# redmod-team/SympGPR

Measured on AMD Instinct MI355X. Metric: Gram-build GB/s + Cholesky fp64 TFLOP/s at N=65536 d=2; |alpha-alpha_ref|/|alpha_ref|, higher is better.
Workload: dtype f64

## Files before the change

### include/sympgpr_probe.h

```cpp
#ifndef SYMPGPR_PROBE_H
#define SYMPGPR_PROBE_H
#include <stddef.h>
#ifdef __cplusplus
extern "C" {
#endif

int sgpr_probe_mfma_f64(int waves_per_simd, int iters, double *tflops);
int sgpr_probe_hbm_write(size_t bytes, int reps, double *gbs);
int sgpr_probe_mfma_clock(int nacc, int waves_per_simd, int iters, double *out3);
int sgpr_probe_gemm(int m, int n, int k, int lower, double *out4);
int sgpr_probe_gemm_debug(int bits);
int sgpr_probe_leaf(double *out8);
int sgpr_probe_lat(double *out8);
int sgpr_probe_xcc(int nblocks, int *host_out);
int sgpr_probe_cumask(const unsigned *mask_words, int nwords, int nblocks, int *host_out);

int sgpr_probe_generated_eval(int family, int which, int m, const double *xa, const double *ya,
                              const double *xb, const double *yb, const double *l, int nl, double *out);

int sgpr_probe_queue_plan(int n, int nworkers, int *starts_out, int max_starts, unsigned *tasks_out, int max_tasks,
                          int *counts);
int sgpr_probe_queue_plan_partial(int n, int nworkers, int nq, int *starts_out, int max_starts, unsigned *tasks_out,
                                  int max_tasks, int *counts);
int sgpr_probe_queue_trace_begin(int max_tasks);
// ... 25 lines not shown
int sgpr_probe_map_team(int ntest, int n0);

int sgpr_probe_trsm_piece(int ticket, int cap, int strips, int out[5]);
int sgpr_probe_trsm_counts(int strips, int cap, unsigned long long out[2]);

int sgpr_probe_census(int na, int threads_a, int lds_a, int spin_a, const unsigned *mask_a, int nwords_a,
                      int nb, int threads_b, int lds_b, int spin_b, const unsigned *mask_b, int nwords_b,
                      unsigned long long *host_out);

int sgpr_probe_strassen_top_plan(int m, int n, int k, int lower, long scratch_doubles, long long *out, int max_records, int *count);
int sgpr_probe_strassen_cfg_plan(int m, int n, int k, int lower, const long cfg[5], long long *out, int max_records, int *count);
int sgpr_probe_strassen_top_scratch(int n, unsigned long long out[2]);
int sgpr_probe_gemm_strassen_top_dev(int m, int n, int k, double alpha, const double *A, size_t lda, const double *B, size_t ldb,
                                     double beta, double *C, size_t ldc, int lower, void *stream);

#ifdef __cplusplus
}
#endif
#endif
```

### sympgpr_amd/_lib.py

```python
import ctypes as C
import os

import numpy as np

FAMILIES = {"A": 0, "B": 1, "C": 2, "D": 3, "USER": 4}
K_KERN, K_DXDX0, K_DYDY0, K_DXDY0 = 0, 1, 2, 3
K_DLX, K_DLY = 4, 8
K_DX, K_DY, K_DX0, K_DY0, K_DXDX0DY0, K_DYDY0DY0, K_DXDY0DY0 = 16, 17, 18, 19, 20, 21, 22
G_QQ, G_PQ, G_QP, G_PP, G_ALL, G_LOWER, G_OCML, G_DLX, G_DLY = 1, 2, 4, 8, 15, 16, 32, 64, 128
FIT_LOWER_ONLY, FIT_REG, FIT_BLOCK_QQ, FIT_BLOCK_PP = 1, 4, 8, 16
MAP_WRAP_Q, MAP_WRAP_P, MAP_EXPLICIT, MAP_LOSS_NEGP = 1, 2, 4, 8
E_ARG, E_NODEVICE, E_HIP, E_NOMEM, E_STATE = -1, -2, -3, -4, -5
LOO_LPD, LOO_PRESS = 0, 1

ABI_VERSION = 5
_dp = C.POINTER(C.c_double)
_vp = C.c_void_p


class SympGPRError(RuntimeError):
    code = None
    detail = ""


# ... 160 lines not shown
                                            C.POINTER(C.c_longlong), C.c_int, C.POINTER(C.c_int)]),
    "sgpr_probe_strassen_rec_plan": (C.c_int, [C.c_int, C.c_int, C.c_int, C.c_int, C.c_long, C.POINTER(C.c_long),
                                               C.POINTER(C.c_longlong), C.c_int, C.POINTER(C.c_int)]),
    "sgpr_probe_strassen_rec_scratch": (C.c_int, [C.c_int, C.POINTER(C.c_ulonglong)]),
    "sgpr_probe_strassen_schedule": (C.c_int, [C.c_int, C.c_int, C.c_int, C.c_int, C.c_long, C.POINTER(C.c_longlong),
                                               C.POINTER(C.c_longlong), C.c_int, C.POINTER(C.c_int)]),
    "sgpr_probe_gemm_strassen_rec_dev": (C.c_int, [C.c_int, C.c_int, C.c_int, C.c_double, C.c_void_p, C.c_size_t, C.c_void_p, C.c_size_t,
                                                   C.c_double, C.c_void_p, C.c_size_t, C.c_int, C.c_void_p]),
    "sgpr_probe_strassen_top_plan": (C.c_int, [C.c_int, C.c_int, C.c_int, C.c_int, C.c_long, C.POINTER(C.c_longlong), C.c_int,
                                               C.POINTER(C.c_int)]),
    "sgpr_probe_strassen_cfg_plan": (C.c_int, [C.c_int, C.c_int, C.c_int, C.c_int, C.POINTER(C.c_long), C.POINTER(C.c_longlong), C.c_int,
                                               C.POINTER(C.c_int)]),
    "sgpr_probe_strassen_top_scratch": (C.c_int, [C.c_int, C.POINTER(C.c_ulonglong)]),
    "sgpr_probe_gemm_strassen_top_dev": (C.c_int, [C.c_int, C.c_int, C.c_int, C.c_double, C.c_void_p, C.c_size_t, C.c_void_p, C.c_size_t,
                                                   C.c_double, C.c_void_p, C.c_size_t, C.c_int, C.c_void_p]),
    "sgpr_probe_gemm_nt4_dev": (C.c_int, [C.c_int, C.c_int, C.c_int, C.c_void_p, C.c_size_t, C.c_void_p, C.c_size_t, C.c_double, C.c_int,
                                          C.POINTER(C.c_void_p), C.POINTER(C.c_size_t), C.POINTER(C.c_double), C.c_void_p]),
    "sgpr_probe_batch_layout": (C.c_int, [C.c_int, C.c_int, C.c_int, C.c_int, C.c_int, C.c_int, C.c_int,
                                          C.POINTER(C.c_ulonglong)]),
    "sgpr_probe_batch_layout_nd_loo": (C.c_int, [C.c_int, C.c_int, C.c_int, C.c_int, C.c_int, C.c_int, C.POINTER(C.c_ulonglong)]),
    "sgpr_probe_census": (C.c_int, [C.c_int, C.c_int, C.c_int, C.c_int, C.POINTER(C.c_uint), C.c_int,
                                    C.c_int, C.c_int, C.c_int, C.c_int, C.POINTER(C.c_uint), C.c_int,
                                    C.POINTER(C.c_ulonglong)]),
}

_LIB = None
_PROBE = None


def load_library():
# ... 87 lines not shown
```

### sympgpr_amd/csrc/chol.h

```cpp
#pragma once
#include "common.h"
#include "strassen.h"
#include "chol_plan.h"

namespace sgpr {

static_assert(cplan::LEAF_ORDER == LEAF, "the planner's leaf order is the kernels'");

struct Ctx {
    double *inv;
    int *dinfo;
    hipStream_t st;
    int la_max = 0;
    int *flags = nullptr;
    void *qws = nullptr;
    bool strassen = false;
    StrassenRec rec;
    StrassenTop top;
};

int potrf_lookahead(int n, double *A, size_t lda, const Ctx &c, int nb, int off0);
int trsm_rec(int m, int n, const double *L, size_t ldl, double *B, size_t ldb, int off, const Ctx &c);
void potrf_clear_queue_mark();

int potrf_queue(int n, double *A, size_t lda, const Ctx &c, int off0);

}
```

### sympgpr_amd/csrc/chol.hip

```cpp
#include <algorithm>
#include <cstdio>
#include <cstdlib>
#include <vector>

#include "cholq.h"
#include "common.h"
#include "strassen.h"
#include "leaf.h"
#include "chol.h"
#include "panel.h"
#include "streams.h"

namespace sgpr {

namespace {

using namespace leaf;
using cplan::split;

unsigned long long *g_panel_dbg = nullptr;

}

int trsm_rec(int m, int n, const double *L, size_t ldl, double *B, size_t ldb, int off, const Ctx &c)
// ... 11 lines not shown
    return trsm_rec(m, n2, L + n1 + (size_t)n1 * ldl, ldl, B + (size_t)n1 * ldb, ldb, off + n1, c);
}

namespace {

int potrf_rec(int n, double *A, size_t lda, int off, const Ctx &c)
{
    if (n <= LEAF) return launch_leaf(n, A, lda, c.inv + (size_t)(off / LEAF) * LEAF * LEAF, c.dinfo, off, (int)LEAF_FACTOR, nullptr, c.st);
    if (n > 4 * LEAF && n <= c.la_max) return potrf_lookahead(n, A, lda, c, 0, off);
    const int n1 = split(n), n2 = n - n1;
    double *A21 = A + n1, *A22 = A + n1 + (size_t)n1 * lda;
    int rc = potrf_rec(n1, A, lda, off, c);
    if (rc) return rc;
    rc = trsm_rec(n2, n1, A, lda, A21, lda, off, c);
    if (rc) return rc;
    if (c.strassen) rc = strassen_top_gemm(n2, n2, n1, -1.0, A21, lda, A21, lda, 1.0, A22, lda, 1, &c.rec, &c.top, c.st);
    else            rc = gemm_nt(n2, n2, n1, -1.0, A21, lda, A21, lda, 1.0, A22, lda, 1, 0, c.st);
    if (rc) return rc;
    return potrf_rec(n2, A22, lda, off + n1, c);
}

}

size_t potrf_workspace(int n) { return cplan::work_layout(n, n <= 0 ? 0 : cholq::ws_bytes(n)).total; }

namespace {

int panel_multi_launch(int pmode, int rows, int w, double *Akk, size_t lda, int goff, const Ctx &cp)
{
    const bool left = pmode != 2, right_in = pmode == 0 || pmode == 3;
    const int below = rows - w;
// ... 183 lines not shown
    const cplan::WorkLayout lay = cplan::work_layout(n, qbytes);
    if (lwork < lay.total) { set_error("potrf: workspace too small"); return SGPR_E_ARG; }
    SGPR_HIP(hipMemsetAsync(dinfo, 0, sizeof(int), st));
    if (n == 0) return 0;
    int *flags = reinterpret_cast<int *>(static_cast<char *>(work) + lay.flags);
    SGPR_HIP(hipMemsetAsync(flags, 0, lay.flag_bytes, st));
    static const int mode = [] { const char *e = getenv("SGPR_POTRF"); return !e ? 0 : (e[0] == 'r' ? 1 : 2); }();
    static const int nb_env = [] { const char *e = getenv("SGPR_POTRF_NB"); return e ? atoi(e) : 0; }();
    const int la_max_env = cplan::la_max_value();
    potrf_clear_queue_mark();
    Ctx c{static_cast<double *>(work), dinfo, st, mode == 1 ? 0 : la_max_env, flags};
    if (qbytes > 0) c.qws = static_cast<char *>(work) + lay.queue;
    c.strassen = true;
    c.rec = strassen_rec_values();
    c.top = strassen_top_values();
    if (n > c.la_max && n > LEAF) {
        size_t need[2];
        potrf_strassen_need(n, need);
        strassen_reserve(need[0], need[1], st);
        strassen_top_reserve(potrf_strassen_top_need(n), st);
    }
    const bool dbg = PANEL_DBG && getenv("SGPR_PANEL_DBG") != nullptr;
    const int T = (n + LEAF - 1) / LEAF;
    if (dbg) {
        (void)hipMalloc((void **)&g_panel_dbg, sizeof(unsigned long long) * 16 * T);
        (void)hipMemset(g_panel_dbg, 0, sizeof(unsigned long long) * 16 * T);
    }
    int rc;
    if (mode == 2 || (nb_env > 0 && mode == 0 && n > 4 * LEAF && n <= c.la_max))
        rc = potrf_lookahead(n, A, lda, c, nb_env > 0 ? nb_env : 0, 0);
// ... 13 lines not shown
```

### sympgpr_amd/csrc/common.h

```cpp
#pragma once
#include <hip/hip_runtime.h>
#include <cstddef>
#include <cstdint>
#include <string>
#include <type_traits>
#include <vector>

#include "../../include/sympgpr_hip.h"

namespace sgpr {

void set_error(const std::string &msg);
double tune(const char *name, double dflt);
void tune_set(const char *name, double v);
int hip_fail(hipError_t e, const char *what, const char *file, int line);

#define SGPR_HIP(call)                                                          \
    do {                                                                        \
        hipError_t e__ = (call);                                                \
        if (e__ != hipSuccess) return ::sgpr::hip_fail(e__, #call, __FILE__, __LINE__); \
    } while (0)

#define SGPR_CHECK_LAUNCH() SGPR_HIP(hipGetLastError())
#define SGPR_HIP_TYPES 1
// ... 84 lines not shown
                    size_t prior_stride, hipStream_t st);
bool family_is_sum(int family);

int gemm_nt(int m, int n, int k, double alpha, const double *A, size_t lda, const double *B,
            size_t ldb, double beta, double *C, size_t ldc, int lower, long diag_off,
            hipStream_t st);
int gemm_nt_bc(int m, int n, int k, double alpha, const double *A, size_t lda, const double *B,
               size_t ldb, double beta, double *C, size_t ldc, int lower, const int *bc5,
               hipStream_t st);
int gemm_nn(int m, int n, int k, double alpha, const double *A, size_t lda, const double *B, size_t ldb,
            double beta, double *C, size_t ldc, hipStream_t st);
int gemm_nt_two(int m, int n, int k, double alpha, const double *A, size_t lda, const double *B, size_t ldb, double beta,
             double *C, size_t ldc, double alpha2, double *C2, size_t ldc2, hipStream_t st);
int gemm_nt_multi(int m, int n, int k, const double *A, size_t lda, const double *B, size_t ldb, double beta, int count,
                  double *const *C, const size_t *ldc, const double *alpha, hipStream_t st);
int gemm_profile_begin();
int gemm_profile_end(double *out12);
int gemm_profile_launches(double *buf, int max_records);
void gemm_set_overlap(int on);
int gemm_nt_diag(int m, int n, int k, double alpha, const double *A, size_t lda, const double *B, size_t ldb,
                 double beta, double *C, size_t ldc, int lower, unsigned long long *stamps, int dbg, hipStream_t st);

constexpr int LEAF = 128;
constexpr int POTRF_HANDOFF_TIMEOUT = -1000001;
constexpr int SOLVE_HANDOFF_TIMEOUT = -1000002;
inline int info_status(int info)
{
    if (info >= 0) return info;
    set_error(info == POTRF_HANDOFF_TIMEOUT ? "potrf: a hand-off inside the panel kernel timed out"
              : info == SOLVE_HANDOFF_TIMEOUT ? "solve: a hand-off between the strips of a triangular solve timed out" : "potrf: internal error");
// ... 134 lines not shown
```

### sympgpr_amd/csrc/gemm_f64.hip

```cpp
#include <algorithm>
#include <atomic>
#include <cstdlib>
#include <mutex>
#include <type_traits>
#include <vector>

#include "common.h"
#include "gemm_tile.h"

namespace sgpr {

namespace {

struct ProfRec { double flop; int big; int m, n, k, lower, overlap; };
struct Prof {
    std::mutex mu;
    std::atomic<bool> on{false};
    std::vector<hipEvent_t> pool;
    std::vector<ProfRec> recs;
    long dropped = 0;
};
constexpr int PROF_POOL = 8192;
Prof g_prof;
thread_local int t_overlap = 0;
// ... 41 lines not shown
}

__global__ __launch_bounds__(512, 2) void gemm_nt4_kernel(const GemmArgs g)
{
    constexpr int BM = 256, BN = 128, LDA_S = BM + PAD, LDB_S = BN + PAD;
    __shared__ double smem[SGPR_GEMM_STAGES * BK * (LDA_S + LDB_S)];
    int tile_r, tile_c;
    if (!tile_of<(SR * BM) / (4 * BN)>(g, tile_r, tile_c)) return;
    const int row0 = tile_r * BM, col0 = tile_c * BN;
    const bool aligned = ((((uintptr_t)g.A | (uintptr_t)g.B) & 15) == 0) && (((g.lda | g.ldb) & 1) == 0);
    const bool fast = aligned && (row0 + BM <= g.m) && (col0 + BN <= g.n) && (g.k % BK == 0);
    if (fast) gemm_body_dma<BM, BN, SGPR_GEMM_STAGES, false, true>(g, smem, tile_r, tile_c);
    else      gemm_body<BM, BN, false, false, false, true>(g, smem, tile_r, tile_c);
}

struct Dst { double *C; size_t ld; double alpha; };

}

int gemm_nt(int m, int n, int k, double alpha, const double *A, size_t lda, const double *B,
            size_t ldb, double beta, double *C, size_t ldc, int lower, long diag_off,
            hipStream_t st)
{
    const int bc[5] = {1, 1, (int)diag_off, 1, 0};
    return gemm_nt_bc(m, n, k, alpha, A, lda, B, ldb, beta, C, ldc, lower, bc, st);
}

static int gemm_launch(int m, int n, int k, double alpha, const double *A, size_t lda, const double *B,
                       size_t ldb, double beta, double *C, size_t ldc, int lower, const int *bc, int transb,
                       hipStream_t st, unsigned long long *stamps = nullptr, int dbg = 0, const Dst *x = nullptr, int nx = 0,
                       bool k4 = false);

static int gemm_chunked(int m, int n, int k, double alpha, const double *A, size_t lda, const double *B,
                        size_t ldb, double beta, double *C, size_t ldc, int lower, const int *bc,
                        hipStream_t st, const Dst *x, int nx, bool k4)
{
    static const int kmax = [] { const char *e = getenv("SGPR_GEMM_KMAX"); return e ? atoi(e) : 8192; }();
    if (kmax >= 128 && k > kmax) {
        const int nchunk = (k + kmax - 1) / kmax;
        const int step = ((k + nchunk - 1) / nchunk + 127) / 128 * 128;
        for (int k0 = 0; k0 < k; k0 += step) {
            const int rc = gemm_launch(m, n, std::min(step, k - k0), alpha, A + (size_t)k0 * lda, lda, B + (size_t)k0 * ldb, ldb,
                                       k0 == 0 ? beta : 1.0, C, ldc, lower, bc, 0, st, nullptr, 0, x, nx, k4);
            if (rc) return rc;
        }
        return 0;
    }
    return gemm_launch(m, n, k, alpha, A, lda, B, ldb, beta, C, ldc, lower, bc, 0, st, nullptr, 0, x, nx, k4);
}

int gemm_nt_bc(int m, int n, int k, double alpha, const double *A, size_t lda, const double *B,
               size_t ldb, double beta, double *C, size_t ldc, int lower, const int *bc,
               hipStream_t st)
{
    return gemm_chunked(m, n, k, alpha, A, lda, B, ldb, beta, C, ldc, lower, bc, st, nullptr, 0, false);
// ... 7 lines not shown
    const Dst x{C2, ldc2, alpha2};
    return gemm_chunked(m, n, k, alpha, A, lda, B, ldb, beta, C, ldc, 0, bc, st, &x, 1, false);
}

int gemm_nt_multi(int m, int n, int k, const double *A, size_t lda, const double *B, size_t ldb, double beta, int count,
                  double *const *C, const size_t *ldc, const double *alpha, hipStream_t st)
{
    const int bc[5] = {1, 1, 0, 1, 0};
    if (count < 2 || count > 4 || !C || !ldc || !alpha) { set_error("gemm_nt_multi: 2 to 4 destinations"); return SGPR_E_ARG; }
    Dst x[3];
    for (int d = 0; d < count; ++d) {
        if (!C[d]) { set_error("gemm_nt_multi: null destination"); return SGPR_E_ARG; }
        if (d) x[d - 1] = Dst{C[d], ldc[d], alpha[d]};
    }
    return gemm_chunked(m, n, k, alpha[0], A, lda, B, ldb, beta, C[0], ldc[0], 0, bc, st, x, count - 1, true);
}

static int gemm_launch(int m, int n, int k, double alpha, const double *A, size_t lda, const double *B,
                       size_t ldb, double beta, double *C, size_t ldc, int lower, const int *bc, int transb,
                       hipStream_t st, unsigned long long *stamps, int dbg, const Dst *x, int nx, bool k4)
{
    const bool plain = bc[0] == 1 && bc[1] == 1 && bc[3] == 1 && bc[4] == 0;
    const long diag_off = plain ? bc[2] : 1;
    if (bc[0] < 1 || bc[1] < 1 || bc[3] < 1) { set_error("gemm_nt: bad block-cyclic descriptor"); return SGPR_E_ARG; }
    if (m < 0 || n < 0 || k < 0) { set_error("gemm_nt: negative extent"); return SGPR_E_ARG; }
    if (m == 0 || n == 0) return 0;
    if (lda < (size_t)m || ldb < (size_t)(transb ? k : n) || ldc < (size_t)m) {
        set_error("gemm: leading dimension too small");
        return SGPR_E_ARG;
    }
    if (nx < 0 || nx > 3 || (nx && !x)) { set_error("gemm: bad destination count"); return SGPR_E_ARG; }
    Dst d[3] = {};
    for (int i = 0; i < nx; ++i) {
        d[i] = x[i];
        if (!d[i].C || lower || transb || d[i].ld < (size_t)m) { set_error("gemm: bad second destination"); return SGPR_E_ARG; }
    }
    GemmArgs g{m, n, k, alpha, beta, A, lda, B, ldb, C, ldc, lower, diag_off, transb, stamps, 0, 0, 0, 0, 0, 0,
               0, 0, bc[0], bc[1], bc[2], bc[3], bc[4], dbg, nullptr, d[0].C, d[0].ld, d[0].alpha,
               d[1].C, d[1].ld, d[1].alpha, d[2].C, d[2].ld, d[2].alpha, nx + 1};
    auto set_map = [&](int bm, int bn) {
        g.tiles_m = (m + bm - 1) / bm;
        g.tiles_n = (n + bn - 1) / bn;
        const int SC = (SR * bm) / (4 * bn);
        g.n_sr = (g.tiles_m + SR - 1) / SR;
        g.n_sc = (g.tiles_n + SC - 1) / SC;
        g.tri = (lower && diag_off == 0 && m == n) ? 1 : 0;
        if (g.tri) {
            long full = 0;
            for (int sc = 0; sc < g.n_sc; ++sc) full += std::max(g.n_sr - sc / 4 - 1, 0);
            g.n_full = (int)full;
            g.n_grp = (g.n_sc + 3) / 4;
            g.n_super = g.n_full + 4 * g.n_grp;
        }
        if (!g.tri) g.n_super = g.n_sr * g.n_sc;
        return (unsigned)(((g.n_super + 7) / 8) * 8 * SR * SC);
    };
    int slot = -1;
    ProfRec rec{};
    if (g_prof.on.load(std::memory_order_acquire)) {
        std::lock_guard<std::mutex> lock(g_prof.mu);
        if (g_prof.on.load(std::memory_order_relaxed)) {
            if ((int)g_prof.recs.size() < PROF_POOL) {
                double elems = (double)m * n;
                if (lower && plain) {
                    elems = 0.0;
                    for (int j = 0; j < n; ++j) {
                        long first = (long)j - diag_off;
                        if (first < 0) first = 0;
                        if (first < m) elems += (double)(m - first);
                    }
                } else if (lower) {
// ... 38 lines not shown
    } else {
        const dim3 grid(set_map(128, 128));
        hipLaunchKernelGGL((gemm_nt_kernel<128, 128>), grid, dim3(256), 0, st, g);
    }
    SGPR_CHECK_LAUNCH();
    if (slot >= 0) {
        SGPR_HIP(hipEventRecord(g_prof.pool[2 * slot + 1], st));
        if (rec.big) {
            std::lock_guard<std::mutex> lock(g_prof.mu);
            if (slot < (int)g_prof.recs.size()) g_prof.recs[slot].big = 1;
        }
    }
    return 0;
}

int gemm_nt_diag(int m, int n, int k, double alpha, const double *A, size_t lda, const double *B, size_t ldb,
                 double beta, double *C, size_t ldc, int lower, unsigned long long *stamps, int dbg, hipStream_t st)
{
    const int bc[5] = {1, 1, 0, 1, 0};
    return gemm_launch(m, n, k, alpha, A, lda, B, ldb, beta, C, ldc, lower, bc, 0, st, stamps, dbg);
}

int gemm_nn(int m, int n, int k, double alpha, const double *A, size_t lda, const double *B, size_t ldb,
            double beta, double *C, size_t ldc, hipStream_t st)
{
    const int bc[5] = {1, 1, 0, 1, 0};
    return gemm_launch(m, n, k, alpha, A, lda, B, ldb, beta, C, ldc, 0, bc, 1, st);
}

void gemm_set_overlap(int on) { t_overlap = on; }
// ... 57 lines not shown
```

### sympgpr_amd/csrc/gemm_tile.h

```cpp
#pragma once
#include <type_traits>

#include "common.h"

namespace sgpr {
namespace tile {

typedef double double4_t __attribute__((ext_vector_type(4)));
typedef double double2_t __attribute__((ext_vector_type(2)));

#ifndef SGPR_GEMM_STAGES
#define SGPR_GEMM_STAGES 2
#endif
constexpr int BK = 16;
constexpr int PAD = 16;

struct GemmArgs {
    int m, n, k;
    double alpha, beta;
    const double *A;
    size_t lda;
    const double *B;
    size_t ldb;
    double *C;
// ... 9 lines not shown
    unsigned long long *kdone;
    double *C2;
    size_t ldc2;
    double alpha2;
    double *C3;
    size_t ldc3;
    double alpha3;
    double *C4;
    size_t ldc4;
    double alpha4;
    int ndst;
};

constexpr int SR = 8;
template <int SC>
__device__ __forceinline__ bool tile_of(const GemmArgs &g, int &tile_r, int &tile_c)
{
    const int L = blockIdx.x;
    const int xcd = L & 7, j = L >> 3;
    const int S = (j / (SR * SC)) * 8 + xcd;
    if (S >= g.n_super) return false;
    const int w = j % (SR * SC);
    int sr, sc;
    if (!g.tri) {
        sc = S / g.n_sr;
        sr = S - sc * g.n_sr;
        if (g.lower) sr = (sr + sc) % g.n_sr;
    } else if (S < g.n_full) {
        const int N1 = g.n_sr - 1;
        const double nsr = (double)N1;
        int a = (int)((2.0 * nsr + 1.0 - sqrt((2.0 * nsr + 1.0) * (2.0 * nsr + 1.0) - 2.0 * (double)S)) * 0.5);
        if (a < 0) a = 0;
        while (a > 0 && 4 * (a * N1 - a * (a - 1) / 2) > S) --a;
// ... 1 lines not shown
        const int rem = S - 4 * (a * N1 - a * (a - 1) / 2);
        const int per = N1 - a;
        const int b = rem / per;
        sc = 4 * a + b;
        sr = a + 1 + (rem - b * per);
    } else {
        const int d = S - g.n_full;
        const int b = d / g.n_grp, a = d - b * g.n_grp;
        sc = 4 * a + b;
        sr = a;
    }
    tile_r = sr * SR + (w % SR);
    tile_c = sc * SC + (w / SR);
    return tile_r < g.tiles_m && tile_c < g.tiles_n;
}

template <int BR, int THREADS, bool FAST>
__device__ __forceinline__ void load_tile(const double *P, size_t ld, int row0,
                                          int k0, int rows, int kmax, int tid,
                                          double2_t (&reg)[BR * BK / (2 * THREADS)])
{
    constexpr int PASSES = BR * BK / (2 * THREADS);
#pragma unroll
    for (int p = 0; p < PASSES; ++p) {
        const int e = p * THREADS + tid;
        const int r = 2 * (e % (BR / 2));
        const int kc = e / (BR / 2);
        if constexpr (FAST) {
            const double *src = P + (size_t)(row0 + r) + (size_t)(k0 + kc) * ld;
            reg[p] = *reinterpret_cast<const double2_t *>(src);
// ... 534 lines not shown
```

### sympgpr_amd/csrc/probe.hip

```cpp
#include <algorithm>
#include <cstdlib>
#include <vector>

#include "cholq.h"
#include "common.h"
#include "strassen.h"
#include "../../include/sympgpr_probe.h"
#include "generated/pair_generated.h"
#include "nd_eval.h"

namespace sgpr {
namespace {
typedef double double4_t __attribute__((ext_vector_type(4)));
typedef double double2_t __attribute__((ext_vector_type(2)));

template <int NACC>
__global__ __launch_bounds__(256) void mfma_clock_kernel(int iters, double *out, unsigned long long *stamps)
{
    double4_t acc[NACC];
    const double a = 1.0 + threadIdx.x * 1e-9, b = 1.0 - threadIdx.x * 1e-9;
#pragma unroll
    for (int i = 0; i < NACC; ++i) acc[i] = double4_t{0.0, 0.0, 0.0, 0.0};
    const unsigned long long t0 = __builtin_amdgcn_s_memtime(), r0 = __builtin_amdgcn_s_memrealtime();
    for (int it = 0; it < iters; ++it) {
// ... 570 lines not shown
    for (size_t i = 0; out && i < plan.size() && (int)(i / STRASSEN_REC) < max_records; ++i) out[i] = plan[i];
    return 0;
}
extern "C" int sgpr_probe_strassen_top_scratch(int n, unsigned long long out[2])
{
    if (n < 0 || !out) { set_error("probe_strassen_top_scratch: bad arguments"); return SGPR_E_ARG; }
    out[0] = potrf_strassen_top_need(n);
    out[1] = 2 * out[0];
    return 0;
}
extern "C" int sgpr_probe_gemm_strassen_top_dev(int m, int n, int k, double alpha, const double *A, size_t lda, const double *B, size_t ldb,
                                                double beta, double *C, size_t ldc, int lower, void *stream)
{
    return strassen_top_gemm(m, n, k, alpha, A, lda, B, ldb, beta, C, ldc, lower, nullptr, nullptr, static_cast<hipStream_t>(stream));
}
static int probe_batch_layout(const char *entry, bool nd_loo, int path, int mode, int d, int reg, int nbatch, int n_pts, int nhyp,
                              unsigned long long out[24])
{
    const long n = d ? 2L * d * n_pts : reg ? (long)n_pts : 2L * n_pts;
    if (path < 0 || path > 1 || mode < 0 || mode > 3 || (path && mode == 3) || d < 0 || d > 3 || (d && (reg || (mode > 1 && !nd_loo))) ||
        nbatch < 1 || n_pts < 1 || nhyp < 1 || (path ? n <= 256 || n > 2048 : n > 256) || !out) {
        set_error(std::string(entry) + ": bad arguments");
        return SGPR_E_ARG;
    }
    const BatchLayout l = batch_layout(path, mode, d, reg, nbatch, n_pts, nhyp);
    const size_t v[24] = {(size_t)l.chunk, l.nacc, l.o_x, l.o_y, l.o_z, l.o_kc, l.o_no, l.in_bytes, l.o_al, l.o_nll, l.o_info, l.out_bytes,
                          l.o_A, l.o_inv, l.o_fl, l.o_fl2, l.o_r, l.o_pub, l.o_st, l.o_part, l.scr_bytes,
                          sizeof(KConst), sizeof(nd::NdConst), l.flag_bytes};
    for (int i = 0; i < 24; ++i) out[i] = v[i];
    return 0;
// ... 72 lines not shown
```

### sympgpr_amd/csrc/strassen.h

```cpp
#pragma once
#include <algorithm>
#include <cstddef>
#include <string>
#include <vector>

#include "../../include/sympgpr_hip.h"

namespace sgpr {

void set_error(const std::string &msg);
double tune(const char *name, double dflt);

constexpr int STRASSEN_REC = 16;
enum { PLAN_SUM = 1, PLAN_PROD = 2, PLAN_CLASSIC = 3 };
int strassen_plan(int m, int n, int k, int lower, long smin, long kslab, size_t scratch_doubles, std::vector<long long> &out);

enum { PLAN2_SUM = 4, PLAN2_PROD = 5 };
int strassen_outer_plan(int m, int n, int k, int lower, long smin, long kslab, long smin2, long kslab2, size_t scratch_doubles,
                   std::vector<long long> &out);
struct StrassenCfg { long smin = -1, kslab = -1, smin2 = -1, kslab2 = -1, smin_under = -1; };
template <typename T> void cfg_to_words(const StrassenCfg &c, T *w)
{
    w[0] = (T)c.smin; w[1] = (T)c.kslab; w[2] = (T)c.smin2; w[3] = (T)c.kslab2; w[4] = (T)c.smin_under;
}
// ... 9 lines not shown
StrassenRec strassen_rec_values();
StrassenCfg strassen_rec_cfg(const StrassenRec &v, int k, int lower);
int strassen_rec_plan(int m, int n, int k, int lower, long cfg_out[5], size_t scratch_doubles, std::vector<long long> &out);

constexpr int SCHED_REC = 32;
int strassen_schedule(int m, int n, int k, int lower, long long cap_doubles, long long info[12], std::vector<long long> &out);

enum { PLAN3_SUM = 6, PLAN3_ZERO = 7, PLAN3_PROD = 8, PLAN3_ACC = 9, PLAN3_PASS = 10 };
struct StrassenTop { long smin3 = 0, kslab3 = 0, kslab3_short = 0; };
StrassenTop strassen_top_values();
int strassen_top_plan(int m, int n, int k, int lower, const StrassenRec *v, const StrassenTop *t, size_t scratch_doubles,
                      std::vector<long long> &out);
int strassen_cfg_plan(int m, int n, int k, int lower, const long cfg[5], std::vector<long long> &out);
size_t strassen_top_scratch_doubles(int m, int n, int k, int lower, const StrassenRec &v, const StrassenTop &t);

void potrf_strassen_need(int n, size_t out[2]);
size_t potrf_strassen_top_need(int n);

namespace splan {
struct PlanCfg {
    long smin;
    long kslab;
    size_t scratch;
};
struct Plan2Cfg {
    PlanCfg in;
    long smin2;
    long kslab2;
    size_t scratch;
    long smin_under = -1;
// ... 15 lines not shown
SchedCfg sched_cfg_of(const Need2 &nd, size_t cap, bool overlap);
void schedule_of(const std::vector<long long> &plan, const Plan2Cfg &c, const Need2 &nd, const SchedCfg &sc, std::vector<long long> &out);
Need3 top_need(const std::vector<long long> &plan);
int top_buffers_wanted();
}

#ifdef SGPR_HIP_TYPES
int gemm_nt_strassen(int m, int n, int k, double alpha, const double *A, size_t lda, const double *B, size_t ldb, double beta,
                     double *C, size_t ldc, int lower, hipStream_t st);
int gemm_nt_strassen_cfg(int m, int n, int k, double alpha, const double *A, size_t lda, const double *B, size_t ldb, double beta,
                         double *C, size_t ldc, int lower, const StrassenCfg &cfg, hipStream_t st);
int gemm_nt_strassen_rec(int m, int n, int k, double alpha, const double *A, size_t lda, const double *B, size_t ldb, double beta,
                         double *C, size_t ldc, int lower, hipStream_t st);
int strassen_top_gemm(int m, int n, int k, double alpha, const double *A, size_t lda, const double *B, size_t ldb, double beta,
                      double *C, size_t ldc, int lower, const StrassenRec *v, const StrassenTop *t, hipStream_t st);
void strassen_reserve(size_t both, size_t one, hipStream_t st);
void strassen_top_reserve(size_t need, hipStream_t st);
int strassen_trim();
int strassen_sum_streams(hipStream_t caller, int count, hipStream_t *out);
int strassen_top_stream(hipStream_t caller, hipStream_t *out);
#endif

}
```

### sympgpr_amd/csrc/strassen.hip

```cpp
#include <algorithm>
#include <cstdint>
#include <mutex>
#include <vector>

#include "common.h"
#include "gemm_tile.h"
#include "strassen.h"

namespace sgpr {
using namespace splan;

namespace {
using namespace tile;

__global__ __launch_bounds__(256) void block_sum_kernel(int rows, int cols, const double *X, size_t ldx, const double *Y, size_t ldy,
                                                        double sign, double *T)
{
    const int nrc = (rows + 511) / 512, ncg = (cols + 3) / 4;
    const long pieces = (long)nrc * ncg;
    for (long p = blockIdx.x; p < pieces; p += gridDim.x) {
        const int cg = (int)(p / nrc), rc = (int)(p - (long)cg * nrc);
        const int r = rc * 512 + 2 * (int)threadIdx.x;
        if (r >= rows) continue;
        double2_t x[4], y[4];
// ... 137 lines not shown
        s.used = true;
    }
};

struct Join {
    hipStream_t st; int n; hipStream_t side[2]; hipEvent_t ev[2];
    ~Join()
    {
        for (int t = 0; t < n; ++t)
            if (hipEventRecord(ev[t], side[t]) != hipSuccess || hipStreamWaitEvent(st, ev[t], 0) != hipSuccess) {
                (void)hipGetLastError();
                (void)hipStreamSynchronize(side[t]);
            }
    }
};

int run_plan(const long long *recs, size_t nrec, double alpha, Mat A, Mat B, double beta, double *C, size_t ldc, double alpha2,
             double *C2, size_t ldc2, double *SA, double *SB, hipStream_t st, long sum_wgs = SUM_WGS)
{
    for (size_t i = 0; i < nrec; ++i) {
        const long long *r = recs + i * STRASSEN_REC;
        int rc = 0;
        if (r[0] == PLAN_SUM) {
            rc = sum_into(r, A, B, r[1] ? SB : SA, st, sum_wgs);
        } else if (r[0] == PLAN_PROD) {
            const int m = (int)r[7], n = (int)r[8], k = (int)r[9];
            const Mat X = operand_of(r, 0, A, SA), Y = operand_of(r, 1, B, SB);
            const Dests d = dests_of(r + 10, alpha, C, ldc);
            if (C2) {
                const Dests e = dests_of(r + 10, alpha2, C2, ldc2);
// ... 4 lines not shown
                auto add = [&](double *p, size_t l, double a) { cs[cnt] = p; ls[cnt] = l; as[cnt] = a; ++cnt; };
                if (d.C2) add(d.C2, ldc, d.a2);
                add(e.C1, ldc2, e.a1);
                if (e.C2) add(e.C2, ldc2, e.a2);
                if (cnt == 2) rc = gemm_nt_two(m, n, k, as[0], X.p, X.ld, Y.p, Y.ld, 1.0, cs[0], ls[0], as[1], cs[1], ls[1], st);
                else          rc = gemm_nt_multi(m, n, k, X.p, X.ld, Y.p, Y.ld, 1.0, cnt, cs, ls, as, st);
            } else if (d.C2) {
                rc = gemm_nt_two(m, n, k, d.a1, X.p, X.ld, Y.p, Y.ld, 1.0, d.C1, ldc, d.a2, d.C2, ldc, st);
            } else {
                rc = gemm_nt(m, n, k, d.a1, X.p, X.ld, Y.p, Y.ld, 1.0, d.C1, ldc, 0, 0, st);
            }
        } else if (r[0] == PLAN_CLASSIC) {
            const double *Ap = block(A.p, A.ld, r[2], r[3]), *Bp = block(B.p, B.ld, r[4], r[5]);
            if (C2) rc = gemm_nt_two((int)r[6], (int)r[7], (int)r[8], alpha, Ap, A.ld, Bp, B.ld, beta, block(C, ldc, r[9], r[10]), ldc,
                                     alpha2, block(C2, ldc2, r[9], r[10]), ldc2, st);
            else    rc = gemm_nt((int)r[6], (int)r[7], (int)r[8], alpha, Ap, A.ld, Bp, B.ld, beta, block(C, ldc, r[9], r[10]), ldc, (int)r[1], 0, st);
        } else {
            set_error("run_plan: unknown record");
            rc = SGPR_E_ARG;
        }
        if (rc) return rc;
    }
    return 0;
}

int run_schedule(const std::vector<long long> &plan, const Plan2Cfg &c, const Need2 &nd, bool overlap, double alpha, Mat A, Mat B,
                 double beta, double *C, size_t ldc, Scratch &s, hipStream_t st)
{
    Use use(s, st);
    int rc = use.begin();
// ... 217 lines not shown
    const int dev = (!v.on || t.smin3 <= 0 || std::min(lower ? m / 2 : m, lower ? n / 2 : n) / 2 < t.smin3) ? -1 : device_of(st);
    if (dev < 0 || strassen_levels() < 2 || !aligned || beta != 1.0 || (lower && m != n))
        return gemm_nt_strassen_cfg(m, n, k, alpha, A, lda, B, ldb, beta, C, ldc, lower, cfg, st);
    std::vector<long long> plan;
    const int rc = strassen_top_plan(m, n, k, lower, &v, &t, ~(size_t)0, plan);
    if (rc) return rc;
    const Need3 nd = top_need(plan);
    if (nd.total()) {
        Scratch &s = g_scratch[1][dev];
        std::lock_guard<std::mutex> lock(s.mu);
        if (ensure(s, nd.total(), top_buffers_wanted(), top_noscratch())) return run_top(plan, nd, alpha, Mat{A, lda}, Mat{B, ldb}, C, ldc, s, st);
    }
    return gemm_nt_strassen_cfg(m, n, k, alpha, A, lda, B, ldb, beta, C, ldc, lower, cfg, st);
}

}
```

### sympgpr_amd/csrc/strassen_plan.hip

```cpp
#include <cstdlib>
#include <initializer_list>

#include "strassen.h"

namespace sgpr {
using namespace splan;

namespace {
void put(std::vector<long long> &out, std::initializer_list<long long> v)
{
    size_t i = 0;
    for (long long x : v) { out.push_back(x); ++i; }
    for (; i < STRASSEN_REC; ++i) out.push_back(0);
}
long slab_of(long k, const PlanCfg &c)
{
    if (k <= 0 || k % 32 != 0 || c.kslab < 32) return 0;
    const long nslab = (k + c.kslab - 1) / c.kslab;
    const long step = ((k + nslab - 1) / nslab + 31) / 32 * 32;
    const long kmin = std::max(c.smin / 2, 16L);
    const long last = k - (nslab - 1) * step;
    if (last <= 0 || step / 2 < kmin || last / 2 < kmin) return 0;
    return step;
}
// ... 410 lines not shown
    return 0;
}
int strassen_cfg_plan(int m, int n, int k, int lower, const long cfg[5], std::vector<long long> &out)
{
    if (bad_extents(m, n, k, lower) || !cfg) { set_error("strassen_cfg_plan: bad arguments"); return SGPR_E_ARG; }
    outer_plan_of(m, n, k, lower, cfg2_of(cfg_of_words(cfg), ~(size_t)0), out);
    return 0;
}
size_t strassen_top_scratch_doubles(int m, int n, int k, int lower, const StrassenRec &v, const StrassenTop &t)
{
    std::vector<long long> plan;
    if (strassen_levels() < 2 || strassen_top_plan(m, n, k, lower, &v, &t, ~(size_t)0, plan)) return 0;
    return top_need(plan).total();
}

}
```

Before: 84.69.

## Batch Strassen diagonal SYRK blocks into grouped triangular GEMM launches

```diff
diff --git a/include/sympgpr_probe.h b/include/sympgpr_probe.h
--- a/include/sympgpr_probe.h
+++ b/include/sympgpr_probe.h
@@ -63,6 +63,12 @@
 int sgpr_probe_gemm_strassen_top_dev(int m, int n, int k, double alpha, const double *A, size_t lda, const double *B, size_t ldb,
                                      double beta, double *C, size_t ldc, int lower, void *stream);
 
+int sgpr_probe_strassen_tri_plan(int n, int k, long tri_min, long long *out, int max_records, int *count);
+int sgpr_probe_tri_group_map(int G, int h, int *out, int max_tiles, int *count);
+int sgpr_probe_gemm_tri_group_dev(int G, int h, int k, double alpha, const double *const *A, size_t lda, double *const *C, size_t ldc,
+                                  void *stream);
+int sgpr_probe_gemm_strassen_tri_dev(int n, int k, double alpha, const double *A, size_t lda, double *C, size_t ldc, void *stream);
+
 #ifdef __cplusplus
 }
 #endif
diff --git a/sympgpr_amd/_lib.py b/sympgpr_amd/_lib.py
--- a/sympgpr_amd/_lib.py
+++ b/sympgpr_amd/_lib.py
@@ -198,6 +198,12 @@
     "sgpr_probe_strassen_top_scratch": (C.c_int, [C.c_int, C.POINTER(C.c_ulonglong)]),
     "sgpr_probe_gemm_strassen_top_dev": (C.c_int, [C.c_int, C.c_int, C.c_int, C.c_double, C.c_void_p, C.c_size_t, C.c_void_p, C.c_size_t,
                                                    C.c_double, C.c_void_p, C.c_size_t, C.c_int, C.c_void_p]),
+    "sgpr_probe_strassen_tri_plan": (C.c_int, [C.c_int, C.c_int, C.c_long, C.POINTER(C.c_longlong), C.c_int, C.POINTER(C.c_int)]),
+    "sgpr_probe_tri_group_map": (C.c_int, [C.c_int, C.c_int, C.POINTER(C.c_int), C.c_int, C.POINTER(C.c_int)]),
+    "sgpr_probe_gemm_tri_group_dev": (C.c_int, [C.c_int, C.c_int, C.c_int, C.c_double, C.POINTER(C.c_void_p), C.c_size_t,
+                                                C.POINTER(C.c_void_p), C.c_size_t, C.c_void_p]),
+    "sgpr_probe_gemm_strassen_tri_dev": (C.c_int, [C.c_int, C.c_int, C.c_double, C.c_void_p, C.c_size_t, C.c_void_p, C.c_size_t,
+                                                   C.c_void_p]),
     "sgpr_probe_gemm_nt4_dev": (C.c_int, [C.c_int, C.c_int, C.c_int, C.c_void_p, C.c_size_t, C.c_void_p, C.c_size_t, C.c_double, C.c_int,
                                           C.POINTER(C.c_void_p), C.POINTER(C.c_size_t), C.POINTER(C.c_double), C.c_void_p]),
     "sgpr_probe_batch_layout": (C.c_int, [C.c_int, C.c_int, C.c_int, C.c_int, C.c_int, C.c_int, C.c_int,
diff --git a/sympgpr_amd/csrc/chol.h b/sympgpr_amd/csrc/chol.h
--- a/sympgpr_amd/csrc/chol.h
+++ b/sympgpr_amd/csrc/chol.h
@@ -17,6 +17,7 @@
     bool strassen = false;
     StrassenRec rec;
     StrassenTop top;
+    long tri_min = 0;
 };
 
 int potrf_lookahead(int n, double *A, size_t lda, const Ctx &c, int nb, int off0);
diff --git a/sympgpr_amd/csrc/chol.hip b/sympgpr_amd/csrc/chol.hip
--- a/sympgpr_amd/csrc/chol.hip
+++ b/sympgpr_amd/csrc/chol.hip
@@ -49,7 +49,7 @@
     if (rc) return rc;
     rc = trsm_rec(n2, n1, A, lda, A21, lda, off, c);
     if (rc) return rc;
-    if (c.strassen) rc = strassen_top_gemm(n2, n2, n1, -1.0, A21, lda, A21, lda, 1.0, A22, lda, 1, &c.rec, &c.top, c.st);
+    if (c.strassen) rc = strassen_tri_syrk(n2, n1, -1.0, A21, lda, A22, lda, &c.rec, &c.top, c.tri_min, c.st);
     else            rc = gemm_nt(n2, n2, n1, -1.0, A21, lda, A21, lda, 1.0, A22, lda, 1, 0, c.st);
     if (rc) return rc;
     return potrf_rec(n2, A22, lda, off + n1, c);
@@ -263,6 +263,7 @@
     c.strassen = true;
     c.rec = strassen_rec_values();
     c.top = strassen_top_values();
+    c.tri_min = strassen_tri_min();
     if (n > c.la_max && n > LEAF) {
         size_t need[2];
         potrf_strassen_need(n, need);
diff --git a/sympgpr_amd/csrc/common.h b/sympgpr_amd/csrc/common.h
--- a/sympgpr_amd/csrc/common.h
+++ b/sympgpr_amd/csrc/common.h
@@ -122,6 +122,8 @@
              double *C, size_t ldc, double alpha2, double *C2, size_t ldc2, hipStream_t st);
 int gemm_nt_multi(int m, int n, int k, const double *A, size_t lda, const double *B, size_t ldb, double beta, int count,
                   double *const *C, const size_t *ldc, const double *alpha, hipStream_t st);
+int gemm_nt_tri_group(int G, int h, int k, double alpha, const double *const *A, size_t lda, double *const *C, size_t ldc, hipStream_t st);
+int gemm_tri_group_tiles(int G, int h, std::vector<int> &out);
 int gemm_profile_begin();
 int gemm_profile_end(double *out12);
 int gemm_profile_launches(double *buf, int max_records);
diff --git a/sympgpr_amd/csrc/gemm_f64.hip b/sympgpr_amd/csrc/gemm_f64.hip
--- a/sympgpr_amd/csrc/gemm_f64.hip
+++ b/sympgpr_amd/csrc/gemm_f64.hip
@@ -79,6 +79,25 @@
     else      gemm_body<BM, BN, false, false, false, true>(g, smem, tile_r, tile_c);
 }
 
+constexpr int TRI_GROUP_MAX = 16;
+struct TriGroup {
+    int slots;
+    const double *A[TRI_GROUP_MAX];
+    double *C[TRI_GROUP_MAX];
+};
+__global__ __launch_bounds__(512, 2) void gemm_tri_group_kernel(const GemmArgs g0, const TriGroup tg)
+{
+    constexpr int BM = 256, BN = 128, LDA_S = BM + PAD, LDB_S = BN + PAD;
+    __shared__ double smem[SGPR_GEMM_STAGES * BK * (LDA_S + LDB_S)];
+    int grp, tile_r, tile_c;
+    if (!tile_of_group<(SR * BM) / (4 * BN)>(g0, tg.slots, (int)blockIdx.x, grp, tile_r, tile_c)) return;
+    if (tile_r * BM + BM - 1 < tile_c * BN) return;
+    GemmArgs g = g0;
+    g.A = g.B = tg.A[grp];
+    g.C = tg.C[grp];
+    gemm_body_dma<BM, BN, SGPR_GEMM_STAGES>(g, smem, tile_r, tile_c);
+}
+
 struct Dst { double *C; size_t ld; double alpha; };
 
 }
@@ -96,14 +115,20 @@
                        hipStream_t st, unsigned long long *stamps = nullptr, int dbg = 0, const Dst *x = nullptr, int nx = 0,
                        bool k4 = false);
 
+static int k_chunk(int k)
+{
+    static const int kmax = [] { const char *e = getenv("SGPR_GEMM_KMAX"); return e ? atoi(e) : 8192; }();
+    if (kmax < 128 || k <= kmax) return k;
+    const int nchunk = (k + kmax - 1) / kmax;
+    return ((k + nchunk - 1) / nchunk + 127) / 128 * 128;
+}
+
 static int gemm_chunked(int m, int n, int k, double alpha, const double *A, size_t lda, const double *B,
                         size_t ldb, double beta, double *C, size_t ldc, int lower, const int *bc,
                         hipStream_t st, const Dst *x, int nx, bool k4)
 {
-    static const int kmax = [] { const char *e = getenv("SGPR_GEMM_KMAX"); return e ? atoi(e) : 8192; }();
-    if (kmax >= 128 && k > kmax) {
-        const int nchunk = (k + kmax - 1) / kmax;
-        const int step = ((k + nchunk - 1) / nchunk + 127) / 128 * 128;
+    const int step = k_chunk(k);
+    if (step < k) {
         for (int k0 = 0; k0 < k; k0 += step) {
             const int rc = gemm_launch(m, n, std::min(step, k - k0), alpha, A + (size_t)k0 * lda, lda, B + (size_t)k0 * ldb, ldb,
                                        k0 == 0 ? beta : 1.0, C, ldc, lower, bc, 0, st, nullptr, 0, x, nx, k4);
@@ -141,6 +166,25 @@
         if (d) x[d - 1] = Dst{C[d], ldc[d], alpha[d]};
     }
     return gemm_chunked(m, n, k, alpha[0], A, lda, B, ldb, beta, C[0], ldc[0], 0, bc, st, x, count - 1, true);
+}
+
+static unsigned set_tile_map(GemmArgs &g, int bm, int bn)
+{
+    g.tiles_m = (g.m + bm - 1) / bm;
+    g.tiles_n = (g.n + bn - 1) / bn;
+    const int SC = (SR * bm) / (4 * bn);
+    g.n_sr = (g.tiles_m + SR - 1) / SR;
+    g.n_sc = (g.tiles_n + SC - 1) / SC;
+    g.tri = (g.lower && g.diag_off == 0 && g.m == g.n) ? 1 : 0;
+    if (g.tri) {
+        long full = 0;
+        for (int sc = 0; sc < g.n_sc; ++sc) full += std::max(g.n_sr - sc / 4 - 1, 0);
+        g.n_full = (int)full;
+        g.n_grp = (g.n_sc + 3) / 4;
+        g.n_super = g.n_full + 4 * g.n_grp;
+    }
+    if (!g.tri) g.n_super = g.n_sr * g.n_sc;
+    return (unsigned)(((g.n_super + 7) / 8) * 8 * SR * SC);
 }
 
 static int gemm_launch(int m, int n, int k, double alpha, const double *A, size_t lda, const double *B,
@@ -165,23 +209,7 @@
     GemmArgs g{m, n, k, alpha, beta, A, lda, B, ldb, C, ldc, lower, diag_off, transb, stamps, 0, 0, 0, 0, 0, 0,
                0, 0, bc[0], bc[1], bc[2], bc[3], bc[4], dbg, nullptr, d[0].C, d[0].ld, d[0].alpha,
                d[1].C, d[1].ld, d[1].alpha, d[2].C, d[2].ld, d[2].alpha, nx + 1};
-    auto set_map = [&](int bm, int bn) {
-        g.tiles_m = (m + bm - 1) / bm;
-        g.tiles_n = (n + bn - 1) / bn;
-        const int SC = (SR * bm) / (4 * bn);
-        g.n_sr = (g.tiles_m + SR - 1) / SR;
-        g.n_sc = (g.tiles_n + SC - 1) / SC;
-        g.tri = (lower && diag_off == 0 && m == n) ? 1 : 0;
-        if (g.tri) {
-            long full = 0;
-            for (int sc = 0; sc < g.n_sc; ++sc) full += std::max(g.n_sr - sc / 4 - 1, 0);
-            g.n_full = (int)full;
-            g.n_grp = (g.n_sc + 3) / 4;
-            g.n_super = g.n_full + 4 * g.n_grp;
-        }
-        if (!g.tri) g.n_super = g.n_sr * g.n_sc;
-        return (unsigned)(((g.n_super + 7) / 8) * 8 * SR * SC);
-    };
+    auto set_map = [&](int bm, int bn) { return set_tile_map(g, bm, bn); };
     int slot = -1;
     ProfRec rec{};
     if (g_prof.on.load(std::memory_order_acquire)) {
@@ -250,6 +278,75 @@
     return 0;
 }
 
+namespace {
+int tri_group_args(int h, int k, double alpha, size_t lda, size_t ldc, GemmArgs &g)
+{
+    g = GemmArgs{};
+    g.m = g.n = h; g.k = k; g.alpha = alpha; g.beta = 1.0; g.lda = g.ldb = lda; g.ldc = ldc; g.lower = 1;
+    g.lblk = g.lpr = g.lpc = 1; g.ndst = 1;
+    return (int)set_tile_map(g, 256, 128);
+}
+}
+
+int gemm_nt_tri_group(int G, int h, int k, double alpha, const double *const *A, size_t lda, double *const *C, size_t ldc, hipStream_t st)
+{
+    if (G < 0 || h < 0 || k < 0 || (G && (!A || !C))) { set_error("gemm_nt_tri_group: bad arguments"); return SGPR_E_ARG; }
+    if (G == 0 || h == 0) return 0;
+    if (lda < (size_t)h || ldc < (size_t)h) { set_error("gemm: leading dimension too small"); return SGPR_E_ARG; }
+    bool takes = h % 256 == 0 && k > 0 && k % BK == 0 && ((lda | ldc) & 1) == 0;
+    for (int g = 0; g < G; ++g) {
+        if (!A[g] || !C[g]) { set_error("gemm_nt_tri_group: null block"); return SGPR_E_ARG; }
+        takes = takes && ((((uintptr_t)A[g] | (uintptr_t)C[g]) & 15) == 0);
+    }
+    if (!takes) {
+        for (int g = 0; g < G; ++g) {
+            const int rc = gemm_nt(h, h, k, alpha, A[g], lda, A[g], lda, 1.0, C[g], ldc, 1, 0, st);
+            if (rc) return rc;
+        }
+        return 0;
+    }
+    const int step = k_chunk(k);
+    for (int k0 = 0; k0 < k; k0 += step)
+        for (int g0 = 0; g0 < G; g0 += TRI_GROUP_MAX) {
+            const int cnt = std::min(TRI_GROUP_MAX, G - g0), kc = std::min(step, k - k0);
+            GemmArgs g;
+            TriGroup tg{};
+            tg.slots = tri_group_args(h, kc, alpha, lda, ldc, g);
+            for (int i = 0; i < cnt; ++i) { tg.A[i] = A[g0 + i] + (size_t)k0 * lda; tg.C[i] = C[g0 + i]; }
+            int slot = -1;
+            if (g_prof.on.load(std::memory_order_acquire)) {
+                std::lock_guard<std::mutex> lock(g_prof.mu);
+                if (g_prof.on.load(std::memory_order_relaxed)) {
+                    if ((int)g_prof.recs.size() < PROF_POOL) {
+                        slot = (int)g_prof.recs.size();
+                        g_prof.recs.push_back(ProfRec{(double)cnt * 2.0 * kc * (0.5 * h * ((double)h + 1.0)), 1, h, h, kc, 1, t_overlap});
+                    } else {
+                        ++g_prof.dropped;
+                    }
+                }
+            }
+            if (slot >= 0) SGPR_HIP(hipEventRecord(g_prof.pool[2 * slot], st));
+            hipLaunchKernelGGL(gemm_tri_group_kernel, dim3((unsigned)(tg.slots * cnt)), dim3(512), 0, st, g, tg);
+            SGPR_CHECK_LAUNCH();
+            if (slot >= 0) SGPR_HIP(hipEventRecord(g_prof.pool[2 * slot + 1], st));
+        }
+    return 0;
+}
+
+int gemm_tri_group_tiles(int G, int h, std::vector<int> &out)
+{
+    out.clear();
+    if (G < 1 || G > TRI_GROUP_MAX || h < 256 || h % 256 != 0) { set_error("gemm_tri_group_tiles: bad arguments"); return SGPR_E_ARG; }
+    GemmArgs g;
+    const int slots = tri_group_args(h, BK, 1.0, (size_t)h, (size_t)h, g);
+    for (int L = 0; L < slots * G; ++L) {
+        int grp, tr, tc;
+        if (!tile_of_group<4>(g, slots, L, grp, tr, tc) || tr * 256 + 255 < tc * 128) continue;
+        for (int v : {grp, L & 7, tr, tc}) out.push_back(v);
+    }
+    return 0;
+}
+
 int gemm_nt_diag(int m, int n, int k, double alpha, const double *A, size_t lda, const double *B, size_t ldb,
                  double beta, double *C, size_t ldc, int lower, unsigned long long *stamps, int dbg, hipStream_t st)
 {
diff --git a/sympgpr_amd/csrc/gemm_tile.h b/sympgpr_amd/csrc/gemm_tile.h
--- a/sympgpr_amd/csrc/gemm_tile.h
+++ b/sympgpr_amd/csrc/gemm_tile.h
@@ -47,9 +47,8 @@
 
 constexpr int SR = 8;
 template <int SC>
-__device__ __forceinline__ bool tile_of(const GemmArgs &g, int &tile_r, int &tile_c)
-{
-    const int L = blockIdx.x;
+__host__ __device__ __forceinline__ bool tile_of_slot(const GemmArgs &g, int L, int &tile_r, int &tile_c)
+{
     const int xcd = L & 7, j = L >> 3;
     const int S = (j / (SR * SC)) * 8 + xcd;
     if (S >= g.n_super) return false;
@@ -81,6 +80,18 @@
     tile_c = sc * SC + (w / SR);
     return tile_r < g.tiles_m && tile_c < g.tiles_n;
 }
+template <int SC>
+__device__ __forceinline__ bool tile_of(const GemmArgs &g, int &tile_r, int &tile_c)
+{
+    return tile_of_slot<SC>(g, (int)blockIdx.x, tile_r, tile_c);
+}
+template <int SC>
+__host__ __device__ __forceinline__ bool tile_of_group(const GemmArgs &g, int slots, int L, int &grp, int &tile_r, int &tile_c)
+{
+    grp = L / slots;
+    const int id = L - grp * slots;
+    return tile_of_slot<SC>(g, (id & ~7) | ((id + 4 * grp) & 7), tile_r, tile_c);
+}
 
 template <int BR, int THREADS, bool FAST>
 __device__ __forceinline__ void load_tile(const double *P, size_t ld, int row0,
diff --git a/sympgpr_amd/csrc/probe.hip b/sympgpr_amd/csrc/probe.hip
--- a/sympgpr_amd/csrc/probe.hip
+++ b/sympgpr_amd/csrc/probe.hip
@@ -608,6 +608,35 @@
 {
     return strassen_top_gemm(m, n, k, alpha, A, lda, B, ldb, beta, C, ldc, lower, nullptr, nullptr, static_cast<hipStream_t>(stream));
 }
+extern "C" int sgpr_probe_strassen_tri_plan(int n, int k, long tri_min, long long *out, int max_records, int *count)
+{
+    if (!count) { set_error("probe_strassen_tri_plan: bad arguments"); return SGPR_E_ARG; }
+    std::vector<long long> plan;
+    const int rc = strassen_tri_plan(n, k, tri_min, nullptr, plan);
+    if (rc) return rc;
+    *count = (int)(plan.size() / STRASSEN_REC);
+    for (size_t i = 0; out && i < plan.size() && (int)(i / STRASSEN_REC) < max_records; ++i) out[i] = plan[i];
+    return 0;
+}
+extern "C" int sgpr_probe_tri_group_map(int G, int h, int *out, int max_tiles, int *count)
+{
+    if (!count) { set_error("probe_tri_group_map: bad arguments"); return SGPR_E_ARG; }
+    std::vector<int> tiles;
+    const int rc = gemm_tri_group_tiles(G, h, tiles);
+    if (rc) return rc;
+    *count = (int)(tiles.size() / 4);
+    for (size_t i = 0; out && i < tiles.size() && (int)(i / 4) < max_tiles; ++i) out[i] = tiles[i];
+    return 0;
+}
+extern "C" int sgpr_probe_gemm_tri_group_dev(int G, int h, int k, double alpha, const double *const *A, size_t lda, double *const *C,
+                                             size_t ldc, void *stream)
+{
+    return gemm_nt_tri_group(G, h, k, alpha, A, lda, C, ldc, static_cast<hipStream_t>(stream));
+}
+extern "C" int sgpr_probe_gemm_strassen_tri_dev(int n, int k, double alpha, const double *A, size_t lda, double *C, size_t ldc, void *stream)
+{
+    return strassen_tri_syrk(n, k, alpha, A, lda, C, ldc, nullptr, nullptr, -1, static_cast<hipStream_t>(stream));
+}
 static int probe_batch_layout(const char *entry, bool nd_loo, int path, int mode, int d, int reg, int nbatch, int n_pts, int nhyp,
                               unsigned long long out[24])
 {
diff --git a/sympgpr_amd/csrc/strassen.h b/sympgpr_amd/csrc/strassen.h
--- a/sympgpr_amd/csrc/strassen.h
+++ b/sympgpr_amd/csrc/strassen.h
@@ -47,6 +47,12 @@
 int strassen_cfg_plan(int m, int n, int k, int lower, const long cfg[5], std::vector<long long> &out);
 size_t strassen_top_scratch_doubles(int m, int n, int k, int lower, const StrassenRec &v, const StrassenTop &t);
 
+enum { PLAN4_TRI = 11, PLAN4_SQUARE = 12 };
+long strassen_tri_min();
+StrassenCfg strassen_tri_cfg(long n, const StrassenRec &v);
+bool strassen_tri_takes(long n, long k, long tri_min, const StrassenRec &v);
+int strassen_tri_plan(int n, int k, long tri_min, const StrassenRec *v, std::vector<long long> &out);
+
 void potrf_strassen_need(int n, size_t out[2]);
 size_t potrf_strassen_top_need(int n);
 
@@ -92,6 +98,8 @@
                          double *C, size_t ldc, int lower, hipStream_t st);
 int strassen_top_gemm(int m, int n, int k, double alpha, const double *A, size_t lda, const double *B, size_t ldb, double beta,
                       double *C, size_t ldc, int lower, const StrassenRec *v, const StrassenTop *t, hipStream_t st);
+int strassen_tri_syrk(int n, int k, double alpha, const double *A, size_t lda, double *C, size_t ldc, const StrassenRec *v,
+                      const StrassenTop *t, long tri_min, hipStream_t st);
 void strassen_reserve(size_t both, size_t one, hipStream_t st);
 void strassen_top_reserve(size_t need, hipStream_t st);
 int strassen_trim();
diff --git a/sympgpr_amd/csrc/strassen.hip b/sympgpr_amd/csrc/strassen.hip
--- a/sympgpr_amd/csrc/strassen.hip
+++ b/sympgpr_amd/csrc/strassen.hip
@@ -175,6 +175,18 @@
             }
     }
 };
+
+struct TriBlock { const double *A; size_t lda; double *C; size_t ldc; int n, k; double alpha; };
+struct TriCollector { long tri_min; StrassenRec v; std::vector<TriBlock> blocks; };
+thread_local TriCollector *t_tri = nullptr;
+bool tri_collect(int n, int k, double alpha, const double *A, size_t lda, double beta, double *C, size_t ldc)
+{
+    TriCollector *const t = t_tri;
+    const bool aligned = ((((uintptr_t)A | (uintptr_t)C) & 15) == 0) && (((lda | ldc) & 1) == 0);
+    if (!t || beta != 1.0 || !aligned || !strassen_tri_takes(n, k, t->tri_min, t->v)) return false;
+    t->blocks.push_back(TriBlock{A, lda, C, ldc, n, k, alpha});
+    return true;
+}
 
 int run_plan(const long long *recs, size_t nrec, double alpha, Mat A, Mat B, double beta, double *C, size_t ldc, double alpha2,
              double *C2, size_t ldc2, double *SA, double *SB, hipStream_t st, long sum_wgs = SUM_WGS)
@@ -209,6 +221,8 @@
             const double *Ap = block(A.p, A.ld, r[2], r[3]), *Bp = block(B.p, B.ld, r[4], r[5]);
             if (C2) rc = gemm_nt_two((int)r[6], (int)r[7], (int)r[8], alpha, Ap, A.ld, Bp, B.ld, beta, block(C, ldc, r[9], r[10]), ldc,
                                      alpha2, block(C2, ldc2, r[9], r[10]), ldc2, st);
+            else if (r[1] && Ap == Bp && A.ld == B.ld && tri_collect((int)r[6], (int)r[8], alpha, Ap, A.ld, beta, block(C, ldc, r[9], r[10]), ldc))
+                rc = 0;
             else    rc = gemm_nt((int)r[6], (int)r[7], (int)r[8], alpha, Ap, A.ld, Bp, B.ld, beta, block(C, ldc, r[9], r[10]), ldc, (int)r[1], 0, st);
         } else {
             set_error("run_plan: unknown record");
@@ -456,4 +470,42 @@
     return gemm_nt_strassen_cfg(m, n, k, alpha, A, lda, B, ldb, beta, C, ldc, lower, cfg, st);
 }
 
-}
+int strassen_tri_syrk(int n, int k, double alpha, const double *A, size_t lda, double *C, size_t ldc, const StrassenRec *vp,
+                      const StrassenTop *tp, long tri_min, hipStream_t st)
+{
+    const StrassenRec v = vp ? *vp : strassen_rec_values();
+    if (tri_min < 0) tri_min = strassen_tri_min();
+    if (tri_min == 0 || !v.on || t_tri) return strassen_top_gemm(n, n, k, alpha, A, lda, A, lda, 1.0, C, ldc, 1, &v, tp, st);
+    TriCollector col{tri_min, v, {}};
+    t_tri = &col;
+    int rc = strassen_top_gemm(n, n, k, alpha, A, lda, A, lda, 1.0, C, ldc, 1, &v, tp, st);
+    t_tri = nullptr;
+    if (rc) return rc;
+    const bool split = tune("rec_tri_split", 1) != 0;
+    std::vector<char> done(col.blocks.size(), 0);
+    for (size_t i = 0; i < col.blocks.size(); ++i) {
+        if (done[i]) continue;
+        const TriBlock &b = col.blocks[i];
+        std::vector<const double *> As;
+        std::vector<double *> Cs;
+        const int h = split ? b.n / 2 : b.n;
+        for (size_t j = i; j < col.blocks.size(); ++j) {
+            const TriBlock &q = col.blocks[j];
+            if (done[j] || q.n != b.n || q.k != b.k || q.lda != b.lda || q.ldc != b.ldc || q.alpha != b.alpha) continue;
+            done[j] = 1;
+            for (int half = 0; half < (split ? 2 : 1); ++half) {
+                As.push_back(q.A + (size_t)half * h);
+                Cs.push_back(q.C + (size_t)half * h + (size_t)half * h * q.ldc);
+            }
+        }
+        if ((rc = gemm_nt_tri_group((int)As.size(), h, b.k, b.alpha, As.data(), b.lda, Cs.data(), b.ldc, st))) return rc;
+    }
+    for (size_t i = 0; split && i < col.blocks.size(); ++i) {
+        const TriBlock &b = col.blocks[i];
+        const int h = b.n / 2;
+        if ((rc = gemm_nt_strassen_cfg(h, h, b.k, b.alpha, b.A + h, b.lda, b.A, b.lda, 1.0, b.C + h, b.ldc, 0, strassen_tri_cfg(b.n, v), st))) return rc;
+    }
+    return 0;
+}
+
+}
diff --git a/sympgpr_amd/csrc/strassen_plan.hip b/sympgpr_amd/csrc/strassen_plan.hip
--- a/sympgpr_amd/csrc/strassen_plan.hip
+++ b/sympgpr_amd/csrc/strassen_plan.hip
@@ -448,4 +448,36 @@
     return top_need(plan).total();
 }
 
-}
+constexpr long REC_TRI_MIN = 16384;
+long strassen_tri_min() { return std::max(0L, (long)tune("rec_tri_min", (double)REC_TRI_MIN)); }
+StrassenCfg strassen_tri_cfg(long n, const StrassenRec &v)
+{
+    StrassenCfg c;
+    c.smin = c.smin_under = n / 4;
+    c.kslab = v.kslab;
+    c.smin2 = 1L << 40;
+    return c;
+}
+bool strassen_tri_takes(long n, long k, long tri_min, const StrassenRec &v)
+{
+    if (!v.on || strassen_levels() < 2 || tri_min <= 0 || n < tri_min || n % tri_min != 0 || n % 4 != 0 || (n / 4) % 256 != 0) return false;
+    return qualifies(n / 2, n / 2, k, PlanCfg{std::max(128L, n / 4), std::max(32L, v.kslab), ~(size_t)0});
+}
+int strassen_tri_plan(int n, int k, long tri_min, const StrassenRec *vp, std::vector<long long> &out)
+{
+    if (bad_extents(n, n, k, 1)) { set_error("strassen_tri_plan: bad extents"); return SGPR_E_ARG; }
+    const StrassenRec v = vp ? *vp : strassen_rec_values();
+    out.clear();
+    if (!strassen_tri_takes(n, k, tri_min < 0 ? strassen_tri_min() : tri_min, v)) {
+        put(out, {PLAN_CLASSIC, 1, 0, 0, 0, 0, n, n, k, 0, 0});
+        return 0;
+    }
+    const long h = n / 2;
+    put(out, {PLAN4_TRI, 0, h, k});
+    put(out, {PLAN4_TRI, h, h, k});
+    put(out, {PLAN4_SQUARE, h, 0, h, h, k, h, 0});
+    put_cfg(out, 8, strassen_tri_cfg(n, v));
+    return 0;
+}
+
+}
```

Result: no change. 85.41, median of 6 (+0.8%).
